# GregDMeyer/dynamite

Hardware: AMD Instinct MI355X
Metric: matrix-free H|psi> Gamplitudes/s, random-field Heisenberg (higher is better)
Workload: dtype f64 (complex128)

## Files before the change

dynamite_amd/_lib.py:

```python
import ctypes as C
import os

import numpy as np

from . import build as _build

_HERE = os.path.dirname(os.path.abspath(__file__))

i64p = C.POINTER(C.c_int64)
f64p = C.POINTER(C.c_double)
vp = C.c_void_p


class Subspace(C.Structure):
    _fields_ = [("type", C.c_int32), ("L", C.c_int64), ("space", C.c_int64), ("k", C.c_int64),
                ("ld_nchoosek", C.c_int64), ("nchoosek", i64p), ("dim", C.c_int64),
                ("state_map", i64p), ("rmap_indices", i64p), ("rmap_states", i64p), ("vec_swizzle", C.c_int32),
                ("site_perm", C.POINTER(C.c_int8))]


class Partition(C.Structure):
    _fields_ = [("rank", C.c_int32), ("nranks", C.c_int32)]


# ... 113 lines not shown
    "dnm_vec_layout_blocks": (C.c_int, [C.POINTER(Subspace), C.c_int64, i64p, i64p, i64p]),
    "dnm_vec_layout_copy": (C.c_int, [C.POINTER(Subspace), C.POINTER(Partition), vp, vp, C.c_int, vp]),
    "dnm_vec_layout_copy_f64": (C.c_int, [C.POINTER(Subspace), C.POINTER(Partition), vp, vp, C.c_int, vp]),
    "dnm_vec_layout_zero_padding": (C.c_int, [C.POINTER(Subspace), C.POINTER(Partition), vp, vp]),
    "dnm_vec_layout_positions": (C.c_int, [C.POINTER(Subspace), C.POINTER(Partition), C.c_int64, vp, vp, vp]),
    "dnm_vec_layout_positions_host": (C.c_int, [C.POINTER(Subspace), C.POINTER(Partition), C.c_int64, i64p, i64p]),
    "dnm_vec_layout_set_random": (C.c_int, [C.POINTER(Subspace), C.POINTER(Partition), vp, C.c_uint64, vp]),
    "dnm_mat_layouts": (C.c_int, [vp, C.POINTER(C.c_int), C.POINTER(C.c_int)]),
    "dnm_mat_window_split": (C.c_int, [vp, C.POINTER(C.c_int)]),
    "dnm_mat_mult_local_part": (C.c_int, [vp, vp, vp, C.c_int, C.c_int, vp]),
    "dnm_mat_local_part_bits": (C.c_int, [vp, C.POINTER(C.c_int), C.POINTER(C.c_int)]),
    "dnm_mat_mult_window_local": (C.c_int, [vp, vp, vp, vp]),
    "dnm_mat_mult_window_remote": (C.c_int, [vp, vp, C.c_int64, C.c_int64, vp, vp]),
    "dnm_mat_window_local_rows": (C.c_int, [vp, C.c_int64, C.c_int64, C.c_int, C.c_int, C.POINTER(C.c_int64), C.POINTER(C.c_int), vp]),
    "dnm_mat_mult_window_rows": (C.c_int, [vp, vp, C.c_int64, C.c_int64, vp, C.c_int64, C.c_int64, vp]),
    "dnm_mat_destroy": (C.c_int, [vp]),
    "dnm_mat_sizes": (C.c_int, [vp, i64p, i64p, i64p, i64p]),
    "dnm_mat_precompute_diagonal": (C.c_int, [vp, vp]),
    "dnm_mat_get_diagonal": (C.c_int, [vp, f64p, vp]),
    "dnm_mat_mult": (C.c_int, [vp, vp, vp, vp]),
    "dnm_mat_norm_inf": (C.c_int, [vp, f64p, vp]),
    "dnm_mat_set_norm": (C.c_int, [vp, C.c_double]),
    "dnm_mat_plan_describe": (C.c_int, [vp, C.c_char_p, C.c_size_t]),
    "dnm_mat_plan_launches": (C.c_int, [vp, C.POINTER(C.c_int)]),
    "dnm_mat_plan_counts": (C.c_int, [vp] + [C.POINTER(C.c_int)] * 6),
    "dnm_mat_export_dtile": (C.c_int, [vp, C.c_int, C.c_int, f64p, C.c_int64]),
    "dnm_mat_export_tabs": (C.c_int, [vp, C.c_int, C.c_int, vp, C.c_size_t, C.c_int, C.POINTER(C.c_int), f64p, C.c_int64, i64p]),
    "dnm_mat_export_pass": (C.c_int, [vp, C.c_int, C.c_int, vp, C.c_size_t, vp, C.c_size_t, C.c_int,
                                      C.POINTER(C.c_int)]),
    "dnm_mat_export_flip": (C.c_int, [vp, C.c_int, C.c_int, vp, C.c_size_t, C.c_int, C.POINTER(C.c_int),
                                      C.POINTER(C.c_uint32), f64p]),
    "dnm_mat_export_flip_pass": (C.c_int, [vp, C.c_int, C.c_int, vp, C.c_size_t, vp, C.c_size_t, C.c_int,
                                           C.POINTER(C.c_int), f64p, C.c_int64, i64p]),
    "dnm_mat_export_diag_tables": (C.c_int, [vp, C.c_int, C.c_int, f64p, C.c_int64, i64p, f64p, C.c_int64, i64p,
                                             C.POINTER(C.c_uint64), C.POINTER(C.c_int)]),
    "dnm_mat_export_sc3": (C.c_int, [vp, C.c_char_p, vp, C.c_size_t, C.POINTER(C.c_size_t)]),
    "dnm_mat_ownership": (C.c_int, [vp, i64p, i64p]),
    "dnm_mat_column_window": (C.c_int, [vp, i64p, i64p, vp]),
    "dnm_mat_column_chunks": (C.c_int, [vp, C.c_int, C.POINTER(C.c_uint8), C.c_int64, vp]),
    "dnm_mat_mult_window": (C.c_int, [vp, vp, C.c_int64, C.c_int64, vp, vp]),
    "dnm_mat_exchange_plan": (C.c_int, [vp, C.POINTER(C.c_int), C.POINTER(Xfer), C.POINTER(C.c_int),
                                        C.POINTER(Xfer)]),
    "dnm_mat_mult_dot": (C.c_int, [vp, vp, vp, f64p, vp]),
    "dnm_mat_mult_lanczos": (C.c_int, [vp, vp, vp, vp, C.c_double, f64p, vp]),
    "dnm_mat_mult_local": (C.c_int, [vp, vp, vp, vp]),
    "dnm_mat_mult_remote": (C.c_int, [vp, C.c_int32, vp, vp, vp]),
    "dnm_vec_set": (C.c_int, [vp, C.c_int64, C.c_double, C.c_double, vp]),
    "dnm_vec_copy": (C.c_int, [vp, vp, C.c_int64, vp]),
    "dnm_vec_scale": (C.c_int, [vp, C.c_int64, C.c_double, C.c_double, vp]),
    "dnm_vec_axpby": (C.c_int, [vp, vp, C.c_int64, C.c_double, C.c_double, C.c_double, C.c_double, vp]),
    "dnm_vec_dot": (C.c_int, [vp, vp, C.c_int64, f64p, vp]),
    "dnm_vec_norm2": (C.c_int, [vp, C.c_int64, f64p, vp]),
    "dnm_vec_set_random": (C.c_int, [vp, C.c_int64, C.c_uint64, C.c_int64, vp]),
    "dnm_vec_mdot": (C.c_int, [vp, C.c_int64, C.c_int, vp, C.c_int64, f64p, vp]),
    "dnm_vec_maxpy": (C.c_int, [vp, vp, C.c_int64, C.c_int, C.c_int64, f64p, vp]),
    "dnm_vec_basis_update": (C.c_int, [vp, C.c_int64, C.c_int, C.c_int, C.c_int64, f64p, vp]),
    "dnm_workspace_bytes": (C.c_int, [C.POINTER(C.c_size_t)]),
    "dnm_release_workspace": (C.c_int, []),
    "dnm_mat_is_real_packed": (C.c_int, [C.c_void_p, C.POINTER(C.c_int)]),
    "dnm_comm_unique_id": (C.c_int, [C.c_void_p]),
    "dnm_comm_create": (C.c_int, [C.c_void_p, C.c_int, C.c_int, C.POINTER(C.c_void_p)]),
    "dnm_comm_destroy": (C.c_int, [C.c_void_p]),
    "dnm_comm_forget": (C.c_int, [C.c_void_p, C.c_void_p]),
    "dnm_comm_loopback": (C.c_int, [C.c_void_p, C.c_int, C.c_int, C.POINTER(C.c_void_p), C.POINTER(C.c_void_p)]),
    "dnm_comm_allreduce": (C.c_int, [C.c_void_p, C.POINTER(C.c_double), C.c_int, C.c_int]),
    "dnm_mat_mult_partitioned": (C.c_int, [C.c_void_p, C.c_void_p, C.c_void_p, C.c_void_p, C.c_void_p]),
# ... 70 lines not shown
```

dynamite_amd/csrc/mat.cpp:

```cpp
#include "passes.h"
#include "vec_api.h"
#include "row_fused.h"

#include <algorithm>
#include <cstring>

namespace dnm {

static thread_local std::string g_err;

void set_error(const char *fmt, ...) {
  char buf[1024];
  va_list ap;
  va_start(ap, fmt);
  vsnprintf(buf, sizeof(buf), fmt, ap);
  va_end(ap);
  g_err = buf;
}

int DevBuf::alloc(size_t nbytes) {
  release();
  if (nbytes == 0) nbytes = 16;
  DNM_HIP(hipMalloc(&p, nbytes));
  bytes = nbytes;
// ... 93 lines not shown
      dev.nchoosek = (const int64_t *)d_nck.p;
    }
    if (!smap.empty()) {
      DNM_TRY(d_smap.upload(smap.data(), smap.size() * 8));
      DNM_TRY(d_rstates.upload(rstates.data(), rstates.size() * 8));
      dev.state_map = (const int64_t *)d_smap.p;
      dev.rmap_states = (const int64_t *)d_rstates.p;
      if (!rind.empty()) {
        DNM_TRY(d_rind.upload(rind.data(), rind.size() * 8));
        dev.rmap_indices = (const int64_t *)d_rind.p;
      }
      if (!bucket.empty()) {
        DNM_TRY(d_bucket.upload(bucket.data(), bucket.size() * 8));
        dev.bucket = (const int64_t *)d_bucket.p;
      }
    }
  }
  return 0;
}

template <class T>
static int upload_to(DevBuf &buf, const std::vector<T> &v, const T **dev) {
  DNM_TRY(buf.upload(v.data(), v.size() * sizeof(T)));
  *dev = (const T *)buf.p;
  return 0;
}
int PassRecords::upload() {
  DNM_TRY(upload_to(d_quads, quads, &desc.quads));
  if (!dtile.empty()) DNM_TRY(upload_to(d_dtile, dblock.empty() ? dtile : dtile_sections(), &desc.dtile));
  if (!dblock.empty()) DNM_TRY(upload_to(d_dblock, dblock, &desc.dblock));
  if (!tabs.empty()) DNM_TRY(upload_to(d_tabs, tabs, &desc.tabs));
  if (!tabs.empty()) DNM_TRY(upload_to(d_tabvals, tabvals, &desc.tabvals));
  if (is_reduced) DNM_TRY(upload_to(d_flips, flips.empty() ? std::vector<DevFlip>(1) : flips, &flip.recs));
  return 0;
}

static hipStream_t S(void *stream) { return (hipStream_t)stream; }

struct PassCall {
  const void *zinit = nullptr, *zinit2 = nullptr;
  double zscale = 0.0, z2re = 0.0, z2im = 0.0;
  double *dot_out = nullptr;
  uint32_t block_offset = 0;
  unsigned nparts = 1;
};

static int launch_pass(const dnm_mat *A, const PassOnDevice &p, const PassCall &c, const void *x, void *y,
                       const void *xr, hipStream_t st) {
  DevPass d = p.runs().desc;
  d.zinit = c.zinit; d.zscale = c.zscale;
  d.zinit2 = c.zinit2; d.z2re = c.z2re; d.z2im = c.z2im;
  d.dot_out = c.dot_out;
  d.block_offset = c.block_offset;
  return launch_tile_pass(d, d.tile_bits, d.log_rows, (A->flags & DNM_MAT_USE_GLDS) != 0, p.n_eff, x, y, xr, st, c.nparts,
                          p.reduced ? &p.reduced->flip : nullptr);
}

static size_t pass_dot_partials(const dnm_mat *, const PassOnDevice &p) {
  return (size_t)1 << (p.n_eff - p.whole.desc.tile_bits);
}

static int export_lookup(const dnm_mat *A, int remote, int idx, const PassOnDevice **p) {
  DNM_CHECK(A, "null argument");
  const auto &v = remote ? A->remote_passes : A->local_passes;
  DNM_CHECK(idx >= 0 && idx < (int)v.size(), "pass index out of range");
  *p = v[idx].get();
// ... 1142 lines not shown

int dnm_mat_export_tabs(const dnm_mat *A, int remote, int idx, void *tabs_out, size_t tab_bytes, int max_tabs, int *ntabs,
                        double *vals_out, int64_t max_vals, int64_t *nvals) {
  const PassOnDevice *p;
  DNM_CHECK(ntabs && nvals, "null argument");
  DNM_TRY(export_lookup(A, remote, idx, &p));
  *ntabs = (int)p->whole.tabs.size();
  *nvals = (int64_t)p->whole.tabvals.size();
  DNM_TRY(export_copy(p->whole.tabs, tabs_out, tab_bytes, max_tabs, "DevTab", "record"));
  return export_copy(p->whole.tabvals, vals_out, sizeof(double), max_vals, "double", "table");
}

int dnm_mat_export_dtile(const dnm_mat *A, int remote, int idx, double *out, int64_t n) {
  const PassOnDevice *p;
  DNM_CHECK(out, "null argument");
  DNM_TRY(export_lookup(A, remote, idx, &p));
  DNM_CHECK((int64_t)p->whole.dtile.size() == n, "the pass has %zu tabulated diagonal entries, not %lld",
            p->whole.dtile.size(), (long long)n);
  return export_copy(p->whole.dtile, out, sizeof(double), n, "double", "table");
}

int dnm_mat_export_flip(const dnm_mat *A, int remote, int idx, void *flips_out, size_t flip_bytes, int max_flips,
                        int *nflips, uint32_t *loops_out, double *dconst) {
  const PassOnDevice *p;
  DNM_CHECK(nflips, "null argument");
  DNM_TRY(export_lookup(A, remote, idx, &p));
  *nflips = p->reduced ? (int)p->reduced->flips.size() : -1;
  if (!p->reduced) return 0;
  if (loops_out) memcpy(loops_out, p->reduced->flip.loop, sizeof(p->reduced->flip.loop));
  if (dconst) *dconst = p->reduced->flip.dconst;
  return export_copy(p->reduced->flips, flips_out, flip_bytes, max_flips, "DevFlip", "record");
}

int dnm_mat_export_flip_pass(const dnm_mat *A, int remote, int idx, void *desc_out, size_t desc_bytes, void *quads_out,
                             size_t quad_bytes, int max_quads, int *nquads, double *dtile_out, int64_t max_dtile,
                             int64_t *ndtile) {
  const PassOnDevice *p;
  DNM_CHECK(nquads && ndtile, "null argument");
  DNM_TRY(export_lookup(A, remote, idx, &p));
  DNM_CHECK(p->reduced, "the pass has no flip-flop form");
  *ndtile = (int64_t)p->reduced->dtile.size();
  DNM_TRY(export_records(*p->reduced, desc_out, desc_bytes, quads_out, quad_bytes, max_quads, nquads, false));
  return export_copy(p->reduced->dtile, dtile_out, sizeof(double), max_dtile, "double", "table");
}

int dnm_mat_export_diag_tables(const dnm_mat *A, int remote, int idx, double *dblock_out, int64_t max_dblock,
                               int64_t *ndblock, double *dtile_out, int64_t max_dtile, int64_t *ndtile,
                               uint64_t *masks_out, int *nmasks) {
  const PassOnDevice *p;
  DNM_CHECK(ndblock && ndtile && nmasks, "null argument");
  DNM_TRY(export_lookup(A, remote, idx, &p));
  const PassRecords &r = p->runs();
  const bool have = !r.dblock.empty();
  *ndblock = (int64_t)r.dblock.size();
  *ndtile = have ? (int64_t)r.dtile_sections().size() : 0;
  *nmasks = have ? (int)r.desc.dsel_n : 0;
  if (!have) return 0;
  if (masks_out) memcpy(masks_out, r.desc.dsel_mask, sizeof(r.desc.dsel_mask));
  DNM_TRY(export_copy(r.dblock, dblock_out, sizeof(double), max_dblock, "double", "table"));
  return export_copy(r.dtile_sections(), dtile_out, sizeof(double), max_dtile, "double", "table");
}

int dnm_mat_export_sc3(const dnm_mat *A, const char *name, void *out, size_t max_bytes, size_t *nbytes) {
  DNM_CHECK(A && name && nbytes, "null argument");
  DNM_CHECK(A->use_sc3 && A->sc3, "the operator does not run on the SpinConserve layout's passes");
  const Sc3Mat &M = *A->sc3;
// ... 60 lines not shown
```

dynamite_amd/csrc/mat.h:

```cpp
#pragma once

#include <memory>
#include <vector>

#include "dev_buf.h"
#include "kernels.h"
#include "plan.h"
#include "sc3.h"
#include "subspace.h"

namespace dnm {

struct SubOwned {
  SubView host{};
  SubView dev{};
  std::vector<int64_t> nck, smap, rind, rstates, bucket;
  DevBuf d_nck, d_smap, d_rind, d_rstates, d_bucket;
  int init(const dnm_subspace *s, bool want_device);
};
int view_from_c(const dnm_subspace *s, SubView *v);

struct PassRecords {
  DevPass desc{};
  std::vector<DevQuad> quads;
  std::vector<double> dtile;
  std::vector<DevTab> tabs;
  std::vector<double> tabvals;
  bool is_reduced = false;
  std::vector<DevFlip> flips;
  DevFlipPass flip{};
  std::vector<double> dblock, dsect;
  const std::vector<double> &dtile_sections() const { return dsect.empty() ? dtile : dsect; }
  DevBuf d_quads, d_dtile, d_tabs, d_tabvals, d_flips, d_dblock;
  int upload();
};

struct PassOnDevice {
  PassRecords whole;
  std::unique_ptr<PassRecords> reduced;
  PassRecords &runs() { return reduced ? *reduced : whole; }
  const PassRecords &runs() const { return reduced ? *reduced : whole; }
  int partner = -1;
  int n_eff = 0;
  int64_t y_off = 0, src_off = 0;
};

struct FlipBond {
  bool ok = false;
  bool exch = false;
  int b0 = 0, b1 = 0;
  double c = 0.0;
};

int rdm_release_scratch();

}

struct dnm_mat {
  std::vector<int64_t> masks, mask_offsets, signs;
  std::vector<double> real_coeffs;
  dnm::SubOwned left, right;
  int64_t M = 0, N = 0, m_local = 0, n_local = 0;
  int64_t row0 = 0;
  bool sc_pair = false;
  bool use_sc3 = false;
  std::unique_ptr<dnm::Sc3Mat> sc3;
// ... 40 lines not shown
```

dynamite_amd/csrc/matvec_kernels.hip:

```cpp
#include <algorithm>
#include <cstdint>
#include <cstdlib>

#include "kernels.h"

namespace dnm {

typedef double2 c128;

#define GLOBAL_AS __attribute__((address_space(1)))
#define LDS_AS __attribute__((address_space(3)))

typedef double d2v __attribute__((ext_vector_type(2)));

typedef const __attribute__((address_space(4))) DevQuad CQuad;

__device__ __forceinline__ void store_through(c128 *p, double re, double im) {
  d2v v = {re, im};
  asm volatile("global_store_dwordx4 %0, %1, off sc1\n\ts_nop 1" ::"v"(p), "v"(v) : "memory");
}
__device__ __forceinline__ void store_streaming(c128 *p, double re, double im) {
  d2v v = {re, im};
  __builtin_nontemporal_store(v, reinterpret_cast<d2v *>(p));
}
// ... 186 lines not shown
    }
  }
}

template <int R>
__device__ __forceinline__ void flip_fma(double c, const c128 (&xv)[R], double (&ar)[R], double (&ai)[R]) {
#pragma unroll
  for (int k = 0; k < R; ++k) {
    ar[k] = fma(c, xv[k].x, ar[k]);
    ai[k] = fma(c, xv[k].y, ai[k]);
  }
}

template <int R, int LOGNT, bool TBITS>
__device__ __forceinline__ void flip_tile(CFlip *__restrict__ flips, uint32_t b, uint32_t e, double (&ar)[R],
                                          double (&ai)[R], const c128 *tile, uint32_t tid) {
  if (b >= e) return;
  const uint32_t last = e - 1;
  auto rec = [&](uint32_t i) { return flip_rec(flips[i < last ? i : last]); };
  c128 xa[R], xb[R];
  FlipRec f0 = rec(b), f1 = rec(b + 1);
  flip_read<R, LOGNT, TBITS>(f0, tile, tid, xa);
  uint32_t qi = b;
  for (; qi + 1 < e; qi += 2) {
    const FlipRec g0 = rec(qi + 2), g1 = rec(qi + 3);
    flip_read<R, LOGNT, TBITS>(f1, tile, tid, xb);
    flip_fma<R>(f0.c, xa, ar, ai);
    flip_read<R, LOGNT, TBITS>(g0, tile, tid, xa);
    flip_fma<R>(f1.c, xb, ar, ai);
    f0 = g0;
    f1 = g1;
  }
  if (qi < e) flip_fma<R>(f0.c, xa, ar, ai);
}

template <int R, int LOGNT>
__device__ __forceinline__ void flip_gathers(CFlip *__restrict__ flips, uint32_t b, uint32_t m, uint32_t e, double (&ar)[R],
                                             double (&ai)[R], const RowAddr<R> &RA, const c128 *__restrict__ x,
                                             uint32_t tid, uint64_t sbase) {
  for (uint32_t qi = b; qi < m; ++qi) {
    CFlip &F = flips[qi];
    if (!((uint32_t)((sbase >> F.p0) ^ (sbase >> F.p1)) & 1u)) continue;
    const uint32_t xm = F.mask_pos;
    c128 xv[R];
#pragma unroll
    for (int k = 0; k < R; ++k) xv[k] = *RA.at(x, k, xm);
    flip_fma<R>(F.c, xv, ar, ai);
  }
  for (uint32_t qi = m; qi < e; ++qi) {
    CFlip &F = flips[qi];
    const uint32_t xm = F.mask_pos;
    const uint32_t outer = (uint32_t)(sbase >> F.p1) & 1u;
    const uint32_t p0 = F.p0;
    c128 xv[R];
#pragma unroll
    for (int k = 0; k < R; ++k) {
      const uint32_t tc = tid | ((uint32_t)k << LOGNT);
      xv[k] = make_double2(0.0, 0.0);
      if ((((tc >> p0) & 1u) ^ outer) != 0u) xv[k] = *RA.at(x, k, xm);
    }
    flip_fma<R>(F.c, xv, ar, ai);
  }
}

typedef const __attribute__((address_space(4))) DevTab CTab;

// ... 191 lines not shown
    }
  } else {
#pragma unroll
    for (int k = 0; k < R; ++k) ar[k] = ai[k] = 0.0;
  }

  CQuad *__restrict__ quads = (CQuad *)P.quads;

#define DNM_LOOP(LP, KV, CX, GA, KZ) \
  apply_records<R, LOGNT, KV, CX, GA, KZ, PACK>(quads, P.loop[LP], P.loop[LP + 1], ar, ai, tile, RA, x, xr, tid, sbase, skw, P.swz_xor_src)
  if constexpr (GV >= 1) {
    DNM_LOOP(LP_GATHER_REAL, false, false, true, false);
    DNM_LOOP(LP_GATHER_KVAR_REAL, true, false, true, false);
    DNM_LOOP(LP_GATHER_CPLX, false, true, true, false);
    DNM_LOOP(LP_GATHER_KVAR_CPLX, true, true, true, false);
  }
#undef DNM_LOOP
  if constexpr (FLIP)
    flip_gathers<R, LOGNT>((CFlip *)FP.recs, FP.loop[FL_GATHER_U], FP.loop[FL_GATHER_B], FP.loop[FL_GATHER_B + 1], ar, ai, RA,
                           x, tid, sbase);
  c128 *tabl = nullptr;
  if constexpr (TAB) {
    __shared__ __attribute__((aligned(16))) unsigned char tabl_mem[TABL_ENTRIES * 16];
    tabl = reinterpret_cast<c128 *>(tabl_mem);
  }
  if constexpr (TAB)
    apply_tabs<R, LOGNT, true>((CTab *)P.tabs, (const c128 *)P.tabvals, P.tab_loop[1], P.tab_loop[2], ar, ai, tile, RA, x, xr,
                               tid, sbase, skw, P.swz_xor_src, tabl);
  DNM_PH(2, 1);

  static_assert(!DT || (!TAB && !PACK), "no table-driven diagonal on the TAB and PACK instances");
  double dext = 0.0;
  uint32_t dsec = 0;
  if constexpr (DT) {
    dext = ((const __attribute__((address_space(4))) double *)P.dblock)[blockIdx.x + P.block_offset];
#pragma unroll
    for (int i = 0; i < MAXDSEL; ++i) dsec |= ((uint32_t)__popcll(sbase & P.dsel_mask[i]) & 1u) << i;
  } else if (P.has_diag) {
    const uint32_t lane = tid & 63u;
    const uint32_t nterm = (P.dext_end - P.dext_begin) * 4u;
    for (uint32_t t0 = 0; t0 < nterm; t0 += 64u) {
      const uint32_t t = t0 + lane;
      double v = 0.0;
      if (t < nterm) {
        CQuad &Q = quads[P.dext_begin + (t >> 2)];
        const uint32_t j = t & 3u;
        const uint32_t p = (uint32_t)__popcll(sbase & Q.sign_ext[j]) & 1u;
        v = flip_sign(Q.coeff[j], p);
      }
      dext += v;
    }
#pragma unroll
    for (int off = 32; off > 0; off >>= 1) dext += __shfl_xor(dext, off, 64);
  }
  double *cg = nullptr;
  if constexpr (TAB) {
    __shared__ double cg_mem[MAXDGROUPS];
    cg = cg_mem;
    if (P.has_diag) {
      const uint32_t lane = tid & 63u, g0 = P.gbucket[0], g1 = P.gbucket[R];
      for (uint32_t g = g0 + (tid >> 6); g < g1; g += (NT >> 6)) {
        const uint32_t q0 = quads[g].mask_loc, nterm = quads[g].src * 4u;
        double v = 0.0;
        for (uint32_t t0 = 0; t0 < nterm; t0 += 64u) {
          const uint32_t t = t0 + lane;
          if (t < nterm) {
            CQuad &Q = quads[q0 + (t >> 2)];
            const uint32_t j = t & 3u;
            v += flip_sign(Q.coeff[j], (uint32_t)__popcll(sbase & Q.sign_ext[j]) & 1u);
          }
        }
#pragma unroll
        for (int off = 32; off > 0; off >>= 1) v += __shfl_xor(v, off, 64);
        if (lane == 0) cg[g - g0] = v;
      }
    }
  }
  auto diag_part2 = [&]() {
  if constexpr (DT) {
    const double *__restrict__ dsect = P.dtile + ((size_t)dsec << B) + tid;
#pragma unroll
    for (int k = 0; k < R; ++k) {
      const double Dk = dext + dsect[k * NT];
      c128 xs = tile[tid + k * NT];
      ar[k] = fma(Dk, xs.x, ar[k]);
      ai[k] = fma(Dk, xs.y, ai[k]);
    }
  } else if (P.has_diag) {
    double D[R];
#pragma unroll
    for (int j = 0; j < R; ++j) D[j] = 0.0;
    D[0] = dext;
    if constexpr (FLIP) D[0] += FP.dconst;
    double dtab[R];
    if (P.dtile) {
#pragma unroll
      for (int k = 0; k < R; ++k) dtab[k] = P.dtile[tid + k * NT];
    }
#pragma unroll
    for (int j = 0; j < R; ++j)
      for (uint32_t q = P.dbucket[j]; q < P.dbucket[j + 1]; ++q) {
        const uint32_t ns = quads[q].nslots;
        double v = slot_amp(quads[q], 0, tid, sbase);
        if (ns > 1) v += slot_amp(quads[q], 1, tid, sbase);
        if (ns > 2) v += slot_amp(quads[q], 2, tid, sbase);
        if (ns > 3) v += slot_amp(quads[q], 3, tid, sbase);
        D[j] += v;
      }
    if constexpr (TAB) {
      const uint32_t g0 = P.gbucket[0];
#pragma unroll
      for (int j = 0; j < R; ++j)
        for (uint32_t q = P.gbucket[j]; q < P.gbucket[j + 1]; ++q)
          D[j] += flip_sign(cg[q - g0], (uint32_t)__popc(tid & quads[q].sign_tile[0]) & 1u);
    }
#pragma unroll
    for (int h = 1; h < R; h <<= 1) {
#pragma unroll
      for (int i = 0; i < R; ++i) {
        if ((i & h) == 0) {
          double a = D[i], b = D[i | h];
          D[i] = a + b;
          D[i | h] = a - b;
        }
      }
    }
    if (P.dtile) {
#pragma unroll
      for (int k = 0; k < R; ++k) D[k] += dtab[k];
    }
#pragma unroll
    for (int k = 0; k < R; ++k) {
      c128 xs = tile[tid + k * NT];
      ar[k] = fma(D[k], xs.x, ar[k]);
      ai[k] = fma(D[k], xs.y, ai[k]);
    }
  }
  };
  __syncthreads();
  DNM_PRIO_LDS();
  DNM_PH(3, 0);
  diag_part2();

  DNM_PH(4, 0);
#define DNM_LOOP(LP, KV, CX, GA, KZ) \
  apply_records<R, LOGNT, KV, CX, GA, KZ, PACK>(quads, P.loop[LP], P.loop[LP + 1], ar, ai, tile, RA, x, xr, tid, sbase, skw, P.swz_xor_src)
  if constexpr (FLIP) {
    flip_tile<R, LOGNT, true>((CFlip *)FP.recs, FP.loop[FL_TILE_T], FP.loop[FL_TILE_T + 1], ar, ai, tile, tid);
    flip_tile<R, LOGNT, false>((CFlip *)FP.recs, FP.loop[FL_TILE_K], FP.loop[FL_TILE_K + 1], ar, ai, tile, tid);
  }
  DNM_LOOP(LP_TILE_REAL_K0, false, false, false, true);
  DNM_LOOP(LP_TILE_REAL, false, false, false, false);
  DNM_LOOP(LP_TILE_CPLX, false, true, false, false);
  DNM_LOOP(LP_TILE_KVAR_REAL, true, false, false, false);
  DNM_LOOP(LP_TILE_KVAR_CPLX, true, true, false, false);
  if constexpr (GV == 0) {
    DNM_LOOP(LP_GATHER_REAL, false, false, true, false);
    DNM_LOOP(LP_GATHER_KVAR_REAL, true, false, true, false);
    DNM_LOOP(LP_GATHER_CPLX, false, true, true, false);
    DNM_LOOP(LP_GATHER_KVAR_CPLX, true, true, true, false);
  }
#undef DNM_LOOP
  if constexpr (TAB)
    apply_tabs<R, LOGNT, false>((CTab *)P.tabs, (const c128 *)P.tabvals, P.tab_loop[0], P.tab_loop[1], ar, ai, tile, RA, x, xr,
                                tid, sbase, skw, P.swz_xor_src, tabl);

  DNM_PH(5, 0);
  DNM_PRIO_MEM();
  if (late_y) {
    c128 w[R];
#pragma unroll
    for (int k = 0; k < R; ++k) w[k] = load_streaming(RA.at((const c128 *)y, k, yx));
#pragma unroll
    for (int k = 0; k < R; ++k) {
      ar[k] += w[k].x;
      ai[k] += w[k].y;
    }
  }
  DNM_PH(6, 1);
  if (P.cache_policy & 64) {
#pragma unroll
    for (int k = 0; k < R; ++k) store_streaming(RA.at(y, k, yx), ar[k], ai[k]);
// ... 991 lines not shown
```

dynamite_amd/csrc/passes.cpp:

```cpp
#include "passes.h"

#include <algorithm>
#include <cstring>

namespace dnm {

int build_opform(const dnm_mat &A, OpForm *op) {
  const SubView &l = A.left.host, &r = A.right.host;
  const bool par = l.type == DNM_PARITY;
  const int n = par ? l.L - 1 : l.L;
  op->n = n;
  op->masks.clear();
  const uint64_t ones = n >= 64 ? ~0ull : (((uint64_t)1 << n) - 1);
  for (size_t mi = 0; mi < A.masks.size(); ++mi) {
    const uint64_t mask = (uint64_t)A.masks[mi];
    if (par && (parity64(mask) != (l.space ^ r.space))) continue;
    RowMask rm;
    rm.mask = par ? (mask >> 1) : mask;
    for (int64_t t = A.mask_offsets[mi]; t < A.mask_offsets[mi + 1]; ++t) {
      const uint64_t sg = (uint64_t)A.signs[t];
      RowTerm rt;
      rt.is_imag = parity64(mask & sg);
      double c = A.real_coeffs[t];
      uint64_t s2 = sg;
// ... 523 lines not shown
  };
  for (int idx : ps.tile_masks) add_flip(idx, false);
  for (int idx : ps.gather_masks) add_flip(idx, true);
  const RowMask *dm = diagonal_mask(op);
  std::vector<RowTerm> dterms;
  if (dm) dterms = dm->terms;
  double dconst = 0.0;
  bool diag_changed = false;
  if (ps.has_diag)
    for (size_t idx = 0; idx < bonds.size(); ++idx) {
      if (!bonds[idx].exch) continue;
      const double a = 0.5 * bonds[idx].c;
      const uint64_t pair = op.masks[idx].mask;
      auto it = std::find_if(dterms.begin(), dterms.end(), [&](const RowTerm &t) { return t.sign == pair; });
      DNM_CHECK(it != dterms.end(), "internal: an exchange without a ZZ term on its pair");
      if (it->coeff == a) dterms.erase(it);
      else it->coeff -= a;
      dconst -= a;
      diag_changed = true;
    }
  if (!diag_changed && std::find(skip.begin(), skip.end(), 1) == skip.end()) return 0;
  std::unique_ptr<PassRecords> r(new PassRecords());
  r->is_reduced = true;
  r->desc = d;
  DNM_TRY(emit_records(A, ps, *r, dm ? &dterms : nullptr, skip));
  DNM_CHECK(r->tabs.empty() && r->desc.gbucket[MAXR] == r->desc.gbucket[0],
            "internal: the flip-flop form of a pass has table records or grouped diagonal terms");
  for (int c = 0; c < FL_COUNT; ++c) {
    r->flip.loop[c] = (uint32_t)r->flips.size();
    r->flips.insert(r->flips.end(), fl[c].begin(), fl[c].end());
  }
  r->flip.loop[FL_COUNT] = (uint32_t)r->flips.size();
  r->flip.dconst = dconst;
  out->reduced = std::move(r);
  return 0;
}

int build_diag_tables(const dnm_mat &A, PassOnDevice *out) {
  PassRecords &r = out->runs();
  DevPass &d = r.desc;
  const char *e = knob("DNM_DIAG_BLOCK_TABLE");
  if (!d.has_diag || (e && e[0] == '0') || r.dtile.empty() || A.op.packed || !(d.cache_policy & 32)) return 0;
  if (!r.tabs.empty() || d.gbucket[MAXR] > d.gbucket[0]) return 0;
  const int B = d.tile_bits, R = 1 << d.log_rows, nbb = d.n_eff - B;
  if (nbb < 0 || nbb > MAXDBLOCK_BITS) return 0;
  std::vector<uint64_t> sel;
  for (uint32_t q = d.dbucket[0]; q < d.dbucket[R]; ++q)
    for (uint32_t j = 0; j < r.quads[q].nslots; ++j) {
      const uint64_t m = r.quads[q].sign_ext[j];
      if (m && std::find(sel.begin(), sel.end(), m) == sel.end()) sel.push_back(m);
    }
  if ((int)sel.size() > MAXDSEL) return 0;
  r.dblock.resize((size_t)1 << nbb);
  for (uint32_t b = 0; b < ((uint32_t)1 << nbb); ++b) {
    uint64_t base = 0;
    for (int j = 0; j < d.nbseg; ++j)
      base |= (uint64_t)((b >> d.bseg_off[j]) & ((1u << d.bseg_len[j]) - 1u)) << d.bseg_pos[j];
    const uint64_t sbase = d.sign_base | base;
    double v = r.is_reduced ? r.flip.dconst : 0.0;
    for (uint32_t q = d.dext_begin; q < d.dext_end; ++q)
      for (uint32_t j = 0; j < r.quads[q].nslots; ++j)
        v += parity64(sbase & r.quads[q].sign_ext[j]) ? -r.quads[q].coeff[j] : r.quads[q].coeff[j];
    r.dblock[b] = v;
  }
  d.dsel_n = (uint32_t)sel.size();
  for (size_t i = 0; i < sel.size(); ++i) d.dsel_mask[i] = sel[i];
  if (!sel.empty()) {
    const size_t T = (size_t)1 << B;
// ... 20 lines not shown
```

dynamite_amd/csrc/passes.h:

```cpp
#pragma once

#include "mat.h"

namespace dnm {

int build_opform(const dnm_mat &A, OpForm *op);
int pack_opform(OpForm *op);
int build_pass(const dnm_mat &A, const PassSpec &ps, PassOnDevice *out);
void decide_flip_bonds(dnm_mat *A);
int build_flip_pass(const dnm_mat &A, const PassSpec &ps, PassOnDevice *out);
int build_diag_tables(const dnm_mat &A, PassOnDevice *out);

}
```

dynamite_amd/csrc/plan.h:

```cpp
#pragma once

#include <cstdint>
#include <string>
#include <vector>

#include "dnm_common.h"

namespace dnm {

constexpr int MAXSEG = 4;
constexpr int MAXBSEG = 8;
constexpr int MAXSRC = 8;
constexpr int MAXR = 16;

struct RowTerm {
  uint64_t sign;
  double coeff;
  int is_imag;
};

struct RowMask {
  uint64_t mask;
  std::vector<RowTerm> terms;
  bool zero_mask_offdiag = false;
// ... 72 lines not shown
  uint32_t swz_xor_y, swz_xor_src;
  uint32_t block_offset;
  uint32_t pos_tmask;
  const double *dtile;
  const DevTab *tabs;
  const double *tabvals;
  uint32_t tab_loop[3];
  uint32_t pad_tab;
  uint32_t gbucket[MAXR + 1];
  uint32_t pad_g;
  const double *dblock;
  uint32_t dsel_n;
  uint32_t pad_d;
  uint64_t dsel_mask[3];
};
constexpr uint32_t MAXDGROUPS = 64;
constexpr int MAXDSEL = 3;
constexpr int MAXDBLOCK_BITS = 22;

struct DevFlip {
  uint32_t mask_tile;
  uint32_t mask_pos;
  uint32_t p0, p1;
  uint32_t pad[2];
  double c;
};
enum {
  FL_TILE_T = 0,
  FL_TILE_K,
  FL_GATHER_U,
  FL_GATHER_B,
  FL_COUNT
};
struct DevFlipPass {
  const DevFlip *recs;
  uint32_t loop[FL_COUNT + 1];
  uint32_t pad;
  double dconst;
};

struct PassSpec {
  int B = 0;
  int logR = 0;
  int nseg = 0;
  int seg_len[MAXSEG] = {0}, seg_pos[MAXSEG] = {0};
  std::vector<int> tile_masks;
  std::vector<int> gather_masks;
  std::vector<int> gather_src;
  bool has_diag = false;
  bool accumulate = false;
  int partner = -1;
  int n_eff = 0;
  int64_t y_off = 0, src_off = 0;
  uint64_t sign_extra = 0;
  int glen = 0, gpos = 0;
  uint64_t tile_bits() const {
    uint64_t m = 0;
    for (int j = 0; j < nseg; ++j) m |= (((uint64_t)1 << seg_len[j]) - 1) << seg_pos[j];
    return m;
  }
};

struct PlanConfig {
  int B = 12;
  int logR = -1;
  int amin = -1;
  int mode = 2;
  int gbits = -1;
  int Bw = 0, logRw = 0;
  int window_first = -1;
  int gbits_window = -1;
// ... 24 lines not shown
```

include/dynamite_amd.h:

```cpp
#ifndef DYNAMITE_AMD_H
#define DYNAMITE_AMD_H

#include <stddef.h>
#include <stdint.h>

#ifdef __cplusplus
extern "C" {
#endif

const char *dnm_last_error(void);
int dnm_version(void);
int dnm_device_count(int *count);
int dnm_set_device(int device);
int dnm_malloc(void **dptr, size_t bytes);
int dnm_free(void *dptr);
int dnm_memcpy_h2d(void *dst, const void *src, size_t bytes, void *stream);
int dnm_memcpy_d2h(void *dst, const void *src, size_t bytes, void *stream);
int dnm_stream_synchronize(void *stream);

enum { DNM_FULL = 0, DNM_PARITY = 1, DNM_EXPLICIT = 2, DNM_SPIN_CONSERVE = 3 };

typedef struct dnm_subspace {
  int32_t type;
  int64_t L;
// ... 54 lines not shown
int dnm_pm_moments_plan(const dnm_subspace *sub, int *tile_rows, int *panel_rows_log2, int *nworkgroups,
                        size_t *lds_bytes, size_t *scratch_bytes);
int dnm_pm_moments(const void *x, const dnm_subspace *sub, double *out, void *stream);
int dnm_pm_partner_indices(const dnm_subspace *sub, int64_t n, const int64_t *rows, int64_t *out);
int dnm_swap_moments_plan(const dnm_subspace *sub, int nbonds, int *tile_rows, int *panel_rows_log2, int *nworkgroups,
                          size_t *lds_bytes, size_t *scratch_bytes);
int dnm_swap_moments(const void *x, const dnm_subspace *sub, int xparity_sector, int nbonds, const int32_t *bonds,
                     double *out, void *stream);
int dnm_swap_partner_indices(const dnm_subspace *sub, int xparity_sector, int nbonds, const int32_t *bonds, int64_t n,
                             const int64_t *rows, int64_t *idx, int8_t *sign);
int dnm_mat_destroy(dnm_mat *A);
int dnm_mat_sizes(const dnm_mat *A, int64_t *M, int64_t *N, int64_t *m_local, int64_t *n_local);
int dnm_mat_precompute_diagonal(dnm_mat *A, void *stream);
int dnm_mat_get_diagonal(dnm_mat *A, double *diag_host, void *stream);
int dnm_mat_mult(dnm_mat *A, const void *x, void *y, void *stream);
int dnm_mat_norm_inf(dnm_mat *A, double *nrm, void *stream);
int dnm_mat_layouts(const dnm_mat *A, int *left, int *right);
int dnm_mat_is_real_packed(const dnm_mat *A, int *packed);
int dnm_mat_set_norm(dnm_mat *A, double nrm);
int dnm_mat_plan_describe(const dnm_mat *A, char *buf, size_t buflen);
int dnm_mat_plan_launches(const dnm_mat *A, int *n);
int dnm_mat_plan_counts(const dnm_mat *A, int *n_local_passes, int *n_remote_passes, int *tiled,
                        int *B, int *logR, int *n_loc);
int dnm_mat_export_dtile(const dnm_mat *A, int remote, int idx, double *out, int64_t n);
int dnm_mat_export_pass(const dnm_mat *A, int remote, int idx, void *desc_out, size_t desc_bytes,
                        void *quads_out, size_t quad_bytes, int max_quads, int *nquads);
int dnm_mat_export_tabs(const dnm_mat *A, int remote, int idx, void *tabs_out, size_t tab_bytes, int max_tabs, int *ntabs,
                        double *vals_out, int64_t max_vals, int64_t *nvals);
int dnm_mat_export_flip(const dnm_mat *A, int remote, int idx, void *flips_out, size_t flip_bytes, int max_flips,
                        int *nflips, uint32_t *loops_out, double *dconst);
int dnm_mat_export_flip_pass(const dnm_mat *A, int remote, int idx, void *desc_out, size_t desc_bytes, void *quads_out,
                             size_t quad_bytes, int max_quads, int *nquads, double *dtile_out, int64_t max_dtile,
                             int64_t *ndtile);
int dnm_mat_export_diag_tables(const dnm_mat *A, int remote, int idx, double *dblock_out, int64_t max_dblock,
                               int64_t *ndblock, double *dtile_out, int64_t max_dtile, int64_t *ndtile,
                               uint64_t *masks_out, int *nmasks);

int dnm_mat_export_sc3(const dnm_mat *A, const char *name, void *out, size_t max_bytes, size_t *nbytes);

typedef struct {
  int32_t partner;
  int32_t pass_id;
  int64_t offset;
  int64_t count;
} dnm_xfer;
int dnm_mat_exchange_plan(const dnm_mat *A, int *nsend, dnm_xfer *sends ,
                          int *nrecv, dnm_xfer *recvs );
int dnm_mat_mult_dot(dnm_mat *A, const void *x, void *y, double *dot , void *stream);
int dnm_mat_mult_lanczos(dnm_mat *A, const void *x, void *y, const void *z, double b,
                         double *dot , void *stream);
int dnm_mat_mult_sub(dnm_mat *A, const void *x, void *y, const void *z, double b, void *stream);
int dnm_mat_fuses_init(const dnm_mat *A);
int dnm_mat_mult_sub2(dnm_mat *A, const void *x, void *y, const void *z, double b, const void *z2,
                      double c_re, double c_im, void *stream);
int dnm_mat_mult_local(dnm_mat *A, const void *x_local, void *y, void *stream);
int dnm_mat_mult_remote(dnm_mat *A, int32_t recv_index, const void *x_recv,
                        void *y, void *stream);

int dnm_mat_ownership(const dnm_mat *A, int64_t *row0, int64_t *m_local);
int dnm_mat_window_split(const dnm_mat *A, int *supported);
int dnm_mat_mult_local_part(dnm_mat *A, const void *x, void *y, int part, int nparts, void *stream);
int dnm_mat_local_part_bits(const dnm_mat *A, int *top_free_bit, int *gathers);
int dnm_mat_mult_window_local(dnm_mat *A, const void *x_local, void *y_local, void *stream);
int dnm_mat_mult_window_remote(dnm_mat *A, const void *x_window, int64_t win_start, int64_t win_len, void *y_local,
                               void *stream);
int dnm_mat_window_local_rows(dnm_mat *A, int64_t col_lo, int64_t col_hi, int max_ranges, int min_blocks,
// ... 116 lines not shown
```

Baseline: 69.17.

## Classify in-tile flip records by lane/wave/row bits and fold self-diagonal into table

Sorts the in-tile flip-flop records into classes based on whether the flipped bits lie in lane, wave, or row positions, then handles each class with a specialized kernel path. Wave- and row-bit flips are wave-uniform, so they can use scalar-indexed loads and compile-time row pairing instead of per-lane generic gathers. For wave-wave and row pairs it also precomputes a per-wave/row diagonal contribution table (sown) that is added to the diagonal term. This adds extra scalar loads, registers and template code, which may raise register pressure.

```diff
diff --git a/dynamite_amd/_lib.py b/dynamite_amd/_lib.py
--- a/dynamite_amd/_lib.py
+++ b/dynamite_amd/_lib.py
@@ -169,6 +169,8 @@
                                       C.POINTER(C.c_uint32), f64p]),
     "dnm_mat_export_flip_pass": (C.c_int, [vp, C.c_int, C.c_int, vp, C.c_size_t, vp, C.c_size_t, C.c_int,
                                            C.POINTER(C.c_int), f64p, C.c_int64, i64p]),
+    "dnm_mat_export_flip_uniform": (C.c_int, [vp, C.c_int, C.c_int, f64p, C.c_int64, i64p, C.POINTER(C.c_uint32), C.c_int,
+                                              C.POINTER(C.c_int)]),
     "dnm_mat_export_diag_tables": (C.c_int, [vp, C.c_int, C.c_int, f64p, C.c_int64, i64p, f64p, C.c_int64, i64p,
                                              C.POINTER(C.c_uint64), C.POINTER(C.c_int)]),
     "dnm_mat_export_sc3": (C.c_int, [vp, C.c_char_p, vp, C.c_size_t, C.POINTER(C.c_size_t)]),
diff --git a/dynamite_amd/csrc/mat.cpp b/dynamite_amd/csrc/mat.cpp
--- a/dynamite_amd/csrc/mat.cpp
+++ b/dynamite_amd/csrc/mat.cpp
@@ -149,6 +149,8 @@
   if (!tabs.empty()) DNM_TRY(upload_to(d_tabs, tabs, &desc.tabs));
   if (!tabs.empty()) DNM_TRY(upload_to(d_tabvals, tabvals, &desc.tabvals));
   if (is_reduced) DNM_TRY(upload_to(d_flips, flips.empty() ? std::vector<DevFlip>(1) : flips, &flip.recs));
+  if (is_reduced) DNM_TRY(upload_to(d_trecs, trecs.empty() ? std::vector<DevFlip>(1) : trecs, &flip.trecs));
+  if (is_reduced && !sown.empty()) DNM_TRY(upload_to(d_sown, sown, &flip.sown));
   return 0;
 }
 
@@ -1357,6 +1359,22 @@
   return export_copy(p->reduced->flips, flips_out, flip_bytes, max_flips, "DevFlip", "record");
 }
 
+int dnm_mat_export_flip_uniform(const dnm_mat *A, int remote, int idx, double *sown_out, int64_t max_sown, int64_t *nsown,
+                                uint32_t *idx_out, int max_idx, int *nidx) {
+  const PassOnDevice *p;
+  DNM_CHECK(nsown && nidx, "null argument");
+  DNM_TRY(export_lookup(A, remote, idx, &p));
+  *nsown = 0;
+  *nidx = -1;
+  if (!p->reduced) return 0;
+  const PassRecords &r = *p->reduced;
+  const std::vector<uint32_t> uni(r.torder.begin() + r.flip.tloop[FT_WAVE_WAVE], r.torder.end());
+  *nsown = (int64_t)r.sown.size();
+  *nidx = (int)uni.size();
+  DNM_TRY(export_copy(r.sown, sown_out, sizeof(double), max_sown, "double", "table"));
+  return export_copy(uni, idx_out, sizeof(uint32_t), max_idx, "uint32_t", "index");
+}
+
 int dnm_mat_export_flip_pass(const dnm_mat *A, int remote, int idx, void *desc_out, size_t desc_bytes, void *quads_out,
                              size_t quad_bytes, int max_quads, int *nquads, double *dtile_out, int64_t max_dtile,
                              int64_t *ndtile) {
diff --git a/dynamite_amd/csrc/mat.h b/dynamite_amd/csrc/mat.h
--- a/dynamite_amd/csrc/mat.h
+++ b/dynamite_amd/csrc/mat.h
@@ -29,9 +29,12 @@
   bool is_reduced = false;
   std::vector<DevFlip> flips;
   DevFlipPass flip{};
+  std::vector<DevFlip> trecs;
+  std::vector<uint32_t> torder;
+  std::vector<double> sown;
   std::vector<double> dblock, dsect;
   const std::vector<double> &dtile_sections() const { return dsect.empty() ? dtile : dsect; }
-  DevBuf d_quads, d_dtile, d_tabs, d_tabvals, d_flips, d_dblock;
+  DevBuf d_quads, d_dtile, d_tabs, d_tabvals, d_flips, d_dblock, d_trecs, d_sown;
   int upload();
 };
 
diff --git a/dynamite_amd/csrc/matvec_kernels.hip b/dynamite_amd/csrc/matvec_kernels.hip
--- a/dynamite_amd/csrc/matvec_kernels.hip
+++ b/dynamite_amd/csrc/matvec_kernels.hip
@@ -242,6 +242,85 @@
     f1 = g1;
   }
   if (qi < e) flip_fma<R>(f0.c, xa, ar, ai);
+}
+
+template <int R, int LOGNT>
+__device__ __forceinline__ void flip_rows_wk(int J, uint32_t w, double c, const c128 *p, double (&ar)[R], double (&ai)[R]) {
+  constexpr uint32_t NT = 1u << LOGNT;
+  const c128 *ps = p + (w << (LOGNT + J));
+  const double c_lo = w ? c : 0.0, c_hi = w ? 0.0 : c;
+  c128 xv[R / 2];
+#pragma unroll
+  for (int i = 0; i < R / 2; ++i) {
+    const int k0 = ((i >> J) << (J + 1)) | (i & ((1 << J) - 1));
+    xv[i] = ps[(uint32_t)k0 * NT];
+  }
+#pragma unroll
+  for (int i = 0; i < R / 2; ++i) {
+    const int k0 = ((i >> J) << (J + 1)) | (i & ((1 << J) - 1)), k1 = k0 | (1 << J);
+    ar[k0] = fma(c_lo, xv[i].x, ar[k0]);
+    ai[k0] = fma(c_lo, xv[i].y, ai[k0]);
+    ar[k1] = fma(c_hi, xv[i].x, ar[k1]);
+    ai[k1] = fma(c_hi, xv[i].y, ai[k1]);
+  }
+}
+template <int R, int LOGNT>
+__device__ __forceinline__ void flip_rows_kk(int J0, int J1, double c, const c128 *p, double (&ar)[R], double (&ai)[R]) {
+  constexpr uint32_t NT = 1u << LOGNT;
+  c128 xv[R];
+#pragma unroll
+  for (int k = 0; k < R; ++k)
+    if ((((k >> J0) ^ (k >> J1)) & 1) != 0) xv[k] = p[(uint32_t)(k ^ (1 << J0) ^ (1 << J1)) * NT];
+#pragma unroll
+  for (int k = 0; k < R; ++k)
+    if ((((k >> J0) ^ (k >> J1)) & 1) != 0) {
+      ar[k] = fma(c, xv[k].x, ar[k]);
+      ai[k] = fma(c, xv[k].y, ai[k]);
+    }
+}
+
+template <int R, int LOGR, int LOGNT>
+__device__ __forceinline__ void flip_uniform_kk(CFlip *__restrict__ trecs, uint32_t b_kk, uint32_t e, double (&ar)[R],
+                                                double (&ai)[R], const c128 *tile, uint32_t tid) {
+  const c128 *p = tile + tid;
+  uint32_t qi = b_kk;
+#pragma unroll
+  for (int j0 = 0; j0 < LOGR; ++j0)
+#pragma unroll
+    for (int j1 = j0 + 1; j1 < LOGR; ++j1)
+      while (qi < e) {
+        const FlipRec F = flip_rec(trecs[qi]);
+        if ((F.mt >> LOGNT) != ((1u << j0) | (1u << j1))) break;
+        flip_rows_kk<R, LOGNT>(j0, j1, F.c, p, ar, ai);
+        ++qi;
+      }
+}
+
+template <int R, int LOGR, int LOGNT>
+__device__ __forceinline__ void flip_uniform(CFlip *__restrict__ trecs, uint32_t b_ww, uint32_t b_wk, uint32_t b_kk,
+                                             double (&ar)[R], double (&ai)[R], const c128 *tile,
+                                             uint32_t tid, uint32_t wave) {
+  constexpr uint32_t NT = 1u << LOGNT;
+  constexpr uint32_t LB = (uint32_t)FLIP_LANE_BITS;
+  for (uint32_t qi = b_ww; qi < b_wk; ++qi) {
+    const FlipRec F = flip_rec(trecs[qi]);
+    if ((((wave >> (F.p0 - LB)) ^ (wave >> (F.p1 - LB))) & 1u) == 0u) continue;
+    const c128 *p = tile + (tid ^ F.mt);
+    c128 xv[R];
+#pragma unroll
+    for (int k = 0; k < R; ++k) xv[k] = p[k * NT];
+    flip_fma<R>(F.c, xv, ar, ai);
+  }
+  uint32_t qi = b_wk;
+#pragma unroll
+  for (int jj = 0; jj < LOGR; ++jj)
+    while (qi < b_kk) {
+      const FlipRec F = flip_rec(trecs[qi]);
+      if (F.p1 != (uint32_t)(LOGNT + jj)) break;
+      const c128 *p = tile + (tid ^ (F.mt & (NT - 1u)));
+      flip_rows_wk<R, LOGNT>(jj, (wave >> (F.p0 - LB)) & 1u, F.c, p, ar, ai);
+      ++qi;
+    }
 }
 
 template <int R, int LOGNT>
@@ -499,6 +578,22 @@
   static_assert(!DT || (!TAB && !PACK), "no table-driven diagonal on the TAB and PACK instances");
   double dext = 0.0;
   uint32_t dsec = 0;
+  constexpr bool SOWN_EARLY = DT || R <= 4;
+  uint32_t wave = 0;
+  bool uni = false;
+  double sown[R];
+  auto load_sown = [&]() {
+    const __attribute__((address_space(4))) double *so =
+        (const __attribute__((address_space(4))) double *)FP.sown + ((size_t)wave << LOGR);
+#pragma unroll
+    for (int k = 0; k < R; ++k) sown[k] = so[k];
+  };
+  if constexpr (FLIP) {
+    wave = (uint32_t)__builtin_amdgcn_readfirstlane((int)(tid >> FLIP_LANE_BITS));
+    uni = FP.sown != nullptr;
+    if constexpr (SOWN_EARLY)
+      if (uni) load_sown();
+  }
   if constexpr (DT) {
     dext = ((const __attribute__((address_space(4))) double *)P.dblock)[blockIdx.x + P.block_offset];
 #pragma unroll
@@ -548,7 +643,9 @@
     const double *__restrict__ dsect = P.dtile + ((size_t)dsec << B) + tid;
 #pragma unroll
     for (int k = 0; k < R; ++k) {
-      const double Dk = dext + dsect[k * NT];
+      double Dk = dext + dsect[k * NT];
+      if constexpr (FLIP)
+        if (uni) Dk += sown[k];
       c128 xs = tile[tid + k * NT];
       ar[k] = fma(Dk, xs.x, ar[k]);
       ai[k] = fma(Dk, xs.y, ai[k]);
@@ -596,11 +693,27 @@
 #pragma unroll
       for (int k = 0; k < R; ++k) D[k] += dtab[k];
     }
+    if constexpr (FLIP)
+      if (uni) {
+        if constexpr (!SOWN_EARLY) load_sown();
+#pragma unroll
+        for (int k = 0; k < R; ++k) D[k] += sown[k];
+      }
 #pragma unroll
     for (int k = 0; k < R; ++k) {
       c128 xs = tile[tid + k * NT];
       ar[k] = fma(D[k], xs.x, ar[k]);
       ai[k] = fma(D[k], xs.y, ai[k]);
+    }
+  } else if constexpr (FLIP) {
+    if (uni) {
+      if constexpr (!SOWN_EARLY) load_sown();
+#pragma unroll
+      for (int k = 0; k < R; ++k) {
+        c128 xs = tile[tid + k * NT];
+        ar[k] = fma(sown[k], xs.x, ar[k]);
+        ai[k] = fma(sown[k], xs.y, ai[k]);
+      }
     }
   }
   };
@@ -613,8 +726,11 @@
 #define DNM_LOOP(LP, KV, CX, GA, KZ) \
   apply_records<R, LOGNT, KV, CX, GA, KZ, PACK>(quads, P.loop[LP], P.loop[LP + 1], ar, ai, tile, RA, x, xr, tid, sbase, skw, P.swz_xor_src)
   if constexpr (FLIP) {
-    flip_tile<R, LOGNT, true>((CFlip *)FP.recs, FP.loop[FL_TILE_T], FP.loop[FL_TILE_T + 1], ar, ai, tile, tid);
-    flip_tile<R, LOGNT, false>((CFlip *)FP.recs, FP.loop[FL_TILE_K], FP.loop[FL_TILE_K + 1], ar, ai, tile, tid);
+    flip_uniform_kk<R, LOGR, LOGNT>((CFlip *)FP.trecs, FP.tloop[FT_K_K], FP.tloop[FT_COUNT], ar, ai, tile, tid);
+    flip_uniform<R, LOGR, LOGNT>((CFlip *)FP.trecs, FP.tloop[FT_WAVE_WAVE], FP.tloop[FT_WAVE_K], FP.tloop[FT_K_K],
+                                 ar, ai, tile, tid, wave);
+    flip_tile<R, LOGNT, true>((CFlip *)FP.trecs, FP.tloop[FT_LANE_T], FP.tloop[FT_LANE_T + 1], ar, ai, tile, tid);
+    flip_tile<R, LOGNT, false>((CFlip *)FP.trecs, FP.tloop[FT_LANE_K], FP.tloop[FT_LANE_K + 1], ar, ai, tile, tid);
   }
   DNM_LOOP(LP_TILE_REAL_K0, false, false, false, true);
   DNM_LOOP(LP_TILE_REAL, false, false, false, false);
diff --git a/dynamite_amd/csrc/passes.cpp b/dynamite_amd/csrc/passes.cpp
--- a/dynamite_amd/csrc/passes.cpp
+++ b/dynamite_amd/csrc/passes.cpp
@@ -579,8 +579,49 @@
   }
   r->flip.loop[FL_COUNT] = (uint32_t)r->flips.size();
   r->flip.dconst = dconst;
+  build_flip_uniform(r.get());
   out->reduced = std::move(r);
   return 0;
+}
+
+void build_flip_uniform(PassRecords *r) {
+  const int B = r->desc.tile_bits, logR = r->desc.log_rows, lognt = B - logR;
+  const uint32_t lb = (uint32_t)FLIP_LANE_BITS;
+  std::vector<uint32_t> cls[FT_COUNT];
+  for (uint32_t q = r->flip.loop[FL_TILE_T]; q < r->flip.loop[FL_GATHER_U]; ++q) {
+    const DevFlip &f = r->flips[q];
+    int c;
+    if (f.p0 < lb) c = (int)f.p1 < lognt ? FT_LANE_T : FT_LANE_K;
+    else c = (int)f.p1 < lognt ? FT_WAVE_WAVE : ((int)f.p0 < lognt ? FT_WAVE_K : FT_K_K);
+    cls[c].push_back(q);
+  }
+  std::stable_sort(cls[FT_WAVE_K].begin(), cls[FT_WAVE_K].end(),
+                   [&](uint32_t a, uint32_t b) { return r->flips[a].p1 < r->flips[b].p1; });
+  std::stable_sort(cls[FT_K_K].begin(), cls[FT_K_K].end(), [&](uint32_t a, uint32_t b) {
+    const DevFlip &fa = r->flips[a], &fb = r->flips[b];
+    return fa.p0 != fb.p0 ? fa.p0 < fb.p0 : fa.p1 < fb.p1;
+  });
+  r->trecs.clear();
+  r->torder.clear();
+  for (int c = 0; c < FT_COUNT; ++c) {
+    r->flip.tloop[c] = (uint32_t)r->torder.size();
+    r->torder.insert(r->torder.end(), cls[c].begin(), cls[c].end());
+  }
+  r->flip.tloop[FT_COUNT] = (uint32_t)r->torder.size();
+  for (uint32_t q : r->torder) r->trecs.push_back(r->flips[q]);
+  r->sown.clear();
+  if (r->flip.tloop[FT_WAVE_WAVE] == r->flip.tloop[FT_COUNT] || B < (int)lb) return;
+  r->sown.assign((size_t)1 << (B - (int)lb), 0.0);
+  for (uint32_t wave = 0; wave < (1u << (lognt - (int)lb)); ++wave)
+    for (uint32_t k = 0; k < (1u << logR); ++k) {
+      const uint32_t wk = wave | (k << (lognt - (int)lb));
+      double s = 0.0;
+      for (uint32_t i = r->flip.tloop[FT_WAVE_WAVE]; i < r->flip.tloop[FT_COUNT]; ++i) {
+        const DevFlip &f = r->trecs[i];
+        if ((((wk >> (f.p0 - lb)) ^ (wk >> (f.p1 - lb))) & 1u) == 0u) s += f.c;
+      }
+      r->sown[((size_t)wave << logR) | k] = s;
+    }
 }
 
 int build_diag_tables(const dnm_mat &A, PassOnDevice *out) {
diff --git a/dynamite_amd/csrc/passes.h b/dynamite_amd/csrc/passes.h
--- a/dynamite_amd/csrc/passes.h
+++ b/dynamite_amd/csrc/passes.h
@@ -9,6 +9,7 @@
 int build_pass(const dnm_mat &A, const PassSpec &ps, PassOnDevice *out);
 void decide_flip_bonds(dnm_mat *A);
 int build_flip_pass(const dnm_mat &A, const PassSpec &ps, PassOnDevice *out);
+void build_flip_uniform(PassRecords *r);
 int build_diag_tables(const dnm_mat &A, PassOnDevice *out);
 
 }
diff --git a/dynamite_amd/csrc/plan.h b/dynamite_amd/csrc/plan.h
--- a/dynamite_amd/csrc/plan.h
+++ b/dynamite_amd/csrc/plan.h
@@ -128,11 +128,23 @@
   FL_GATHER_B,
   FL_COUNT
 };
+enum {
+  FT_LANE_T = 0,
+  FT_LANE_K,
+  FT_WAVE_WAVE,
+  FT_WAVE_K,
+  FT_K_K,
+  FT_COUNT
+};
+constexpr int FLIP_LANE_BITS = 6;
 struct DevFlipPass {
   const DevFlip *recs;
   uint32_t loop[FL_COUNT + 1];
   uint32_t pad;
   double dconst;
+  const DevFlip *trecs;
+  const double *sown;
+  uint32_t tloop[FT_COUNT + 1];
 };
 
 struct PassSpec {
diff --git a/include/dynamite_amd.h b/include/dynamite_amd.h
--- a/include/dynamite_amd.h
+++ b/include/dynamite_amd.h
@@ -110,6 +110,8 @@
 int dnm_mat_export_flip_pass(const dnm_mat *A, int remote, int idx, void *desc_out, size_t desc_bytes, void *quads_out,
                              size_t quad_bytes, int max_quads, int *nquads, double *dtile_out, int64_t max_dtile,
                              int64_t *ndtile);
+int dnm_mat_export_flip_uniform(const dnm_mat *A, int remote, int idx, double *sown_out, int64_t max_sown, int64_t *nsown,
+                                uint32_t *idx_out, int max_idx, int *nidx);
 int dnm_mat_export_diag_tables(const dnm_mat *A, int remote, int idx, double *dblock_out, int64_t max_dblock,
                                int64_t *ndblock, double *dtile_out, int64_t max_dtile, int64_t *ndtile,
                                uint64_t *masks_out, int *nmasks);
```

Result: no change. 68.97 (-0.3%).
